# Bhasha-Open/Akshar

Hardware: AMD Instinct MI355X
Metric: MB of raw UTF-8 tokenized/sec @1 GPU (+ tokens/s); bit-exact vs CPU ref (higher is better)
Workload: dtype u8

## Files before the change

akshar_amd/csrc/ak_tile.h:

```cpp
#pragma once
#include <stddef.h>

#include "ak_dev.h"
#include "ak_ptc.h"
#include "ak_rows.h"
#include "ak_wave.h"

namespace ak {

#ifndef AK_T_BCAP
#define AK_T_BCAP 768
#endif
constexpr int T_BCAP = AK_T_BCAP;
constexpr int T_MAXR = 16;
#ifndef AK_TILE_UNIT
#define AK_TILE_UNIT 64
#endif
#ifndef AK_KNOCKOUT
#define AK_KNOCKOUT 0
#endif
#ifndef AK_TILE_WIDE
#define AK_TILE_WIDE 29
#endif
constexpr int TW_D1 = 1, TW_N = 4, TW_F = 8, TW_NS = 16;
// ... 388 lines not shown
    const bool dcand = ok && !(h & H_STABLE) && nfc_d_cand(h, hprev);
    uint32_t first = 0u;
    bool cand2 = false;
    if (lcand) {
        const uint32_t pi = hot_index(ppcp);
        const uint32_t pph = H[pi < HOT_N ? pi : 0u];
        cand2 = pi < HOT_N && (pph >> H_CCC_SHIFT) == 0u && !(pph & H_EXP);
        first = ppcp;
    } else if (dcand) {
        const uint2 pr = prop_global(pcp);
        cand2 = ((pr.y >> 16) & 7u) == 2u;
        first = cand2 ? AK_UT_DECOMP[pr.y >> 19] : 0u;
    }
    lok = cand2 && compose_pair<NF_UCD>(first, cp) == 0u;
    if ((lane == 0 && carry_cmp) || (lane == 1 && (carry_cmp & 2u))) lok = false;
#if AK_D2_SWAP
    const uint32_t hpp = w_prev(hprev, H_ROWSTART);
    const uint32_t hnx = w_next(h, H_ROWSTART);
    const bool ncmp = w_next((uint32_t)cmp, 1u) != 0u;
    const bool pok = w_prev((uint32_t)ok, 0u) != 0u;
    const uint32_t cm = h >> H_CCC_SHIFT, cpv = hprev >> H_CCC_SHIFT;
    const uint32_t cnx = (hnx & (H_STABLE | H_EXP)) ? 0u : (hnx >> H_CCC_SHIFT);
    bool scand = ok && pok && !cmp && !pfb && !lok && lane >= 1 && lane <= 62 && !(h & (H_STABLE | H_DECOMP)) &&
                 hprev != H_ROWSTART && !(hprev & (H_STABLE | H_DECOMP)) && cm != 0u && cm < cpv &&
                 (hpp == H_ROWSTART || (hpp >> H_CCC_SHIFT) == 0u) && (cnx == 0u || cnx >= cpv) && !ncmp &&
                 !(lane == 1 && (carry_cmp & 2u));
    if (w_ballot(scand && (h & H_SECOND))) {
        if (scand && (h & H_SECOND) && compose_pair<NF_UCD>(ppcp, cp) != 0u) scand = false;
    }
    const uint32_t mvn = w_next(mv), mvp = w_prev(mv, 0u);
    const bool sfirst = w_next((uint32_t)scand) != 0u;
    if (scand) {
        mv = mvp;
        lok = true;
    }
    if (sfirst) mv = mvn;
#endif
    const uint32_t cnext = w_next(cmp ? (cmv | 0x10000u) : 0u);
    if (cmp) mv = 0u;
    if (cnext) mv = cnext & 0xFFFFu;
    if (cmp && lane == 0) M.v[vpos - 1] = (uint16_t)cmv;
    const uint32_t cmp_hi = (uint32_t)(w_ballot(cmp) >> 62);
    return D2Exact{hp, hprev, mv, cmp_hi, pfb, lok};
}

template <int BCAP, class Mem, bool NFCD = false, int WIDE = 0>
__device__ __forceinline__ TileRows tile_front(const RowArgs &a, uint64_t r0, uint64_t rend, const uint32_t *H, Mem &M,
                                               bool raw = false) {
    const bool RAW = NFCD && raw;
    const int lane = w_lane();
    const int nr0 = (int)(rend - r0);
    const uint64_t myoff = lane <= nr0 ? a.offs[r0 + lane] : 0ull;
    const uint64_t S0 = w_bcast(myoff, 0);
    const bool fits = lane >= 1 && lane <= nr0 && (myoff - S0) <= (uint64_t)BCAP;
    const int k = w_popc(w_ballot(fits));
    const int nr = k ? k : 1;
    const uint64_t S1 = w_bcast(myoff, k);
    const uint64_t a0 = S0 & ~15ull;
    {
        const uint64_t nblk = (S1 - a0 + 15) / 16;
        const uint4 *src = (const uint4 *)(a.in) + a0 / 16;
        uint4 *dst = (uint4 *)M.bytes;
        for (uint64_t b = (uint64_t)lane; b < nblk; b += 64) dst[b] = src[b];
    }
    const uint64_t nextoff = w_shfl(myoff, lane + 1);
    if (lane < nr) {
        M.fb[lane] = lane >= k ? 1 : 0;
        M.rowend[lane] = (uint16_t)(nextoff - a0);
    }
    w_sync();

    if (AK_KNOCKOUT == 8) return TileRows{k, nr, S0, a0, 0u};
    uint16_t *P = M.w;
    uint32_t np = 0;
    bool swept = false;
    if constexpr ((WIDE & TW_D1) != 0) {
        static_assert(BCAP + 16 + 128 <= 32 * 32 && sizeof(M.v) >= 32 * 4, "the row-start bitmap: 32 dwords of V");
        const int s = lane < k ? (int)(myoff - a0) : 0;
        const uint32_t fbyte = M.bytes[s];
        swept = k > 0 && !w_ballot(lane < k && (nextoff == myoff || (fbyte & 0xC0u) == 0x80u));
        if (swept) {
            uint32_t *BM = (uint32_t *)M.v;
            if (lane < 32) BM[lane] = 0u;
            w_sync();
            if (lane < k) w_lds_or32(&BM[s >> 5], 1u << (s & 31));
            w_sync();
            const int s0 = (int)(S0 - a0), end = (int)(S1 - a0);
            const uint16_t *B2 = (const uint16_t *)M.bytes;
            uint16_t *dummy = M.w + (sizeof(M.w) / 2 - 64) + lane;
            for (int base = s0 & ~1; base < end; base += 128) {
                const int p0 = base + 2 * lane;
                const int pc = p0 < (end & ~1) ? p0 : (end & ~1);
                const uint32_t bb = B2[pc >> 1];
                const uint32_t mk = (BM[p0 >> 5] >> (p0 & 31)) & 3u;
                const bool l0 = p0 >= s0 && p0 < end && (bb & 0xC0u) != 0x80u;
                const bool l1 = p0 + 1 < end && (bb & 0xC000u) != 0x8000u;
                const uint32_t m0 = mk & 1u, m1 = mk >> 1;
                const uint32_t n0 = (uint32_t)l0 + m0;
                uint32_t tot;
                const uint32_t at = np + w_exscan(n0 + (uint32_t)l1 + m1, &tot);
                *(m0 ? &P[at] : dummy) = 0x8000u;
                *(l0 ? &P[at + m0] : dummy) = (uint16_t)p0;
                *(m1 ? &P[at + n0] : dummy) = 0x8000u;
                *(l1 ? &P[at + n0 + m1] : dummy) = (uint16_t)(p0 + 1);
                np += tot;
            }
        }
    }
    for (int i = 0; i < (swept ? 0 : k); ++i) {
        const int s = (int)(w_bcast(myoff, i) - a0), e = (int)(w_bcast(myoff, i + 1) - a0);
        if (lane == 0) P[np] = 0x8000u;
        ++np;
        bool bad_row = false;
        for (int base = s; base < e; base += 64) {
            const int p = base + lane;
            const bool in = p < e;
            const uint32_t b = in ? M.bytes[p] : 0u;
            const bool lead = in && (b & 0xC0u) != 0x80u;
            if (w_ballot(in && !lead && p == s)) { bad_row = true; break; }
            const uint64_t LM = w_ballot(lead);
            if (lead) P[np + w_rank(LM)] = (uint16_t)p;
            np += (uint32_t)w_popc(LM);
        }
        if (bad_row && lane == 0) M.fb[i] = 1;
    }
    w_sync();

    if (AK_KNOCKOUT == 9) return TileRows{k, nr, S0, a0, 0u};
    static_assert(sizeof(M.w) / 2 - 64 >= (size_t)(BCAP + T_MAXR + 1), "D2 dummy slots overlap P");
    uint16_t *dummy = M.w + (sizeof(M.w) / 2 - 64) + lane;
    uint32_t vpos = 0;
    {
        uint32_t carry_h = H_ROWSTART, rows = 0;
        uint32_t carry_cmp = 0;
        const uint32_t plast = np ? np - 1 : 0;
        const uint32_t hn_deva = H[0x093Cu - 0x900u + HOT_LO], hn_beng = H[0x09BCu - 0x900u + HOT_LO];
        for (uint32_t c0 = 0; c0 < np; c0 += 64) {
            const uint32_t c = c0 + lane;
            const bool in = c < np;
            const uint32_t ent0 = P[in ? c : plast];
            const uint32_t nent0 = P[c + 1 < np ? c + 1 : plast];
            const uint32_t ent = in ? ent0 : 0x8000u;
            const bool mark = in && (ent & 0x8000u);
            const uint64_t RMK = w_ballot(mark);
            const int row = (int)(rows + w_rank_incl(RMK)) - 1;
            const bool chr = in && !mark;
            const int pos = (int)(ent & 0x7FFFu);
            const int rend = (int)M.rowend[row > 0 ? row : 0];
            const uint32_t cp = decode_word(lds_word(M.bytes, pos), pos, rend);
            const uint32_t nent = c + 1 < np ? nent0 : 0x8000u;
            const int nxt = (nent & 0x8000u) ? rend : (int)nent;
#if AK_D2_BITWISE
            const bool bad = chr & ((cp == 0xFFFFFFFFu) | (pos + utf8_len(cp) != nxt) | (RAW & (cp >= V_SPECIAL)));
#else
            const bool bad = chr && (cp == 0xFFFFFFFFu || pos + utf8_len(cp) != nxt || (RAW && cp >= V_SPECIAL));
#endif
            const uint32_t ci = cp < HOT_LO ? cp : (cp - 0x900u < 0x100u ? cp - 0x900u + HOT_LO : 0u);
            uint32_t hw = H[ci];
#if AK_D2_BITWISE
            const bool cold = chr & !bad & (ci == 0u) & (cp != 0u);
#else
            const bool cold = chr && !bad && ci == 0u && cp != 0u;
#endif
            if (w_ballot(cold)) {
                if (cold) hw = hot_word(cp);
            }
            const uint32_t h = chr ? (bad ? 0u : hw) : H_ROWSTART;
            const bool xp = !RAW && chr && (h & H_EXP);
            uint32_t hp = xp ? ((h & 0xFFFFu) < 0x0980u ? hn_deva : hn_beng) : h;
            uint32_t hprev = w_prev(hp, carry_h);
            uint32_t mv = RAW ? (chr && !bad ? cp : 0u) : (chr ? (h & 0xFFFFu) : 0u);
#if AK_D2_BITWISE
            const bool ok = chr & !bad & !xp;
            const bool t0 = !NFCD && (ok & ((h & H_STABLE) == 0u) & nfc_trig_bf<false>(h, hprev));
            const bool pc = !NFCD && (ok & (hprev != H_ROWSTART) & ((h & H_SECOND) != 0u) & ((hprev & H_FIRST) != 0u));
#else
            const bool ok = chr && !bad && !xp;
            const bool t0 = !NFCD && ok && !(h & H_STABLE) && nfc_trig<false>(h, hprev);
            const bool pc = !NFCD && ok && nfc_pair_cand(h, hprev);
#endif
            uint32_t cmp_hi = 0;
            if (w_ballot(bad || t0 || pc)) {
                bool pfb = false, lok = false;
                if (AK_KNOCKOUT != 15 && !NFCD) {
                    const D2Exact r = d2_exact(M, P, H, c0, rows, vpos, carry_h, carry_cmp, h, cp, ok, chr, hp, hprev, mv);
                    hp = r.hp;
                    hprev = r.hprev;
                    mv = r.mv;
                    pfb = r.pfb;
                    lok = r.lok;
                    cmp_hi = r.cmp_hi;
                }
                const bool trig = bad || pfb || (!NFCD && ok && !(h & H_STABLE) && !lok && nfc_trig<false>(h, hprev));
                if (trig) M.fb[row] = 1;
            }
            const bool two = mark && row > 0;
            const uint32_t cnt = mark ? (two ? 2u : 1u) : (mv ? (xp ? 2u : 1u) : 0u);
            uint32_t tot;
            const uint32_t ex = w_exscan(cnt, &tot);
            uint16_t *d0 = cnt ? &M.v[vpos + ex] : dummy;
            uint16_t *d1 = (two || xp) ? &M.v[vpos + ex + 1] : dummy;
            *d0 = mark ? (two ? V_E : V_B) : (uint16_t)mv;
            *d1 = two ? V_B : (uint16_t)nukta_of(mv);
            vpos += tot;
            rows += (uint32_t)w_popc(RMK);
            carry_h = w_bcast(hp, 63);
            carry_cmp = cmp_hi;
        }
        if (k > 0) {
            if (lane == 0) M.v[vpos] = V_E;
            ++vpos;
        }
    }
    w_sync();
    return TileRows{k, nr, S0, a0, vpos};
}

__device__ __forceinline__ uint4 load_x4(const uint4 *p) {
#ifdef AK_HOST_EMU
    return *p;
#else
    typedef unsigned int u32x4 __attribute__((ext_vector_type(4)));
    const u32x4 v = *(const u32x4 *)p;
    return make_uint4(v.x, v.y, v.z, v.w);
#endif
}
__device__ __forceinline__ uint32_t ptc_probe(const BpeDev &m, bool cand, uint32_t n, const uint32_t q[7]) {
    const uint4 *tab = (const uint4 *)m.ptc;
    const uint32_t h = akp::ptc_hash(n, q[0], q[1], q[2], q[3], q[4], q[5], q[6]);
    const uint32_t s1 = akp::ptc_slot1(h, m.ptc_mask), s2 = akp::ptc_slot2(h, m.ptc_mask);
    const uint4 a = load_x4(tab + 2 * s1);
    bool m1 = cand & (((a.x >> 16) & 15u) == n) & (a.y == q[0]) & (a.z == q[1]) & (a.w == q[2]);
    if (w_ballot(m1 && n > 6)) {
        const uint4 b = load_x4(tab + 2 * s1 + 1);
        m1 = m1 & ((n <= 6) | ((b.x == q[3]) & (b.y == q[4]) & (b.z == q[5]) & (b.w == q[6])));
    }
    uint32_t res = m1 ? (a.x & 0xFFFFu) : 0xFFFFFFFFu;
    const bool try2 = cand & !m1 & ((a.x & akp::PTC_FLAG) != 0u);
    if (w_ballot(try2)) {
        const uint4 c = load_x4(tab + 2 * s2);
        bool m2 = try2 & (((c.x >> 16) & 15u) == n) & (c.y == q[0]) & (c.z == q[1]) & (c.w == q[2]);
        if (w_ballot(m2 && n > 6)) {
            const uint4 d = load_x4(tab + 2 * s2 + 1);
            m2 = m2 & ((n <= 6) | ((d.x == q[3]) & (d.y == q[4]) & (d.z == q[5]) & (d.w == q[6])));
        }
        res = m2 ? (c.x & 0xFFFFu) : res;
    }
    return res;
}


#ifndef AK_POOL_NCLASS
#define AK_POOL_NCLASS 1
#endif
constexpr int POOL_NCLASS = AK_POOL_NCLASS;
constexpr uint32_t POOL_RING = 320;
constexpr uint32_t POOL_CAP = POOL_NCLASS * POOL_RING;
#ifndef AK_POOL_INLINE
#define AK_POOL_INLINE 0
#endif
constexpr uint32_t POOL_U4 = POOL_CAP * (AK_POOL_INLINE ? 3u : 1u);
constexpr uint32_t STAGE_DEAD = 0xFFFFFFFFu;
static_assert(POOL_NCLASS == 1 || POOL_NCLASS == 4 || POOL_NCLASS == 8, "pool classes");
__device__ __forceinline__ uint32_t pool_class(uint32_t n) {
    if (POOL_NCLASS == 1) return 0u;
    if (POOL_NCLASS == 4) return n <= 3u ? 0u : n <= 5u ? 1u : n <= 8u ? 2u : 3u;
    return n <= 7u ? n - 2u : (n <= 9u ? 6u : 7u);
}

__device__ __forceinline__ uint4 load_l2(const uint4 *p) {
#ifdef AK_HOST_EMU
    return *p;
#else
    typedef unsigned int u32x4 __attribute__((ext_vector_type(4)));
    const u32x4 v = __builtin_nontemporal_load((const u32x4 *)p);
    return make_uint4(v.x, v.y, v.z, v.w);
#endif
}
__device__ __forceinline__ uint32_t load_l2(const uint32_t *p) {
#ifdef AK_HOST_EMU
    return *p;
#else
    return __builtin_nontemporal_load(p);
#endif
}

__device__ __forceinline__ void merge_rounds(const BpeDev &m, uint16_t *sym, uint16_t *rk16, uint32_t &alive,
                                             PassClock &pc) {
    for (;;) {
        if (AK_KNOCKOUT == 2) break;
        uint32_t e[WREG / 2];
        {
            const uint4 *r4 = (const uint4 *)rk16;
            const uint4 x0 = r4[0], x1 = r4[1];
            e[0] = x0.x; e[1] = x0.y; e[2] = x0.z; e[3] = x0.w; e[4] = x1.x; e[5] = x1.y; e[6] = x1.z; e[7] = x1.w;
        }
        const uint32_t m01 = pk_min_u16(e[0], e[1]), m23 = pk_min_u16(e[2], e[3]);
        const uint32_t m45 = pk_min_u16(e[4], e[5]), m67 = pk_min_u16(e[6], e[7]);
        const uint32_t mv = pk_min_u16(pk_min_u16(m01, m23), pk_min_u16(m45, m67));
        const uint32_t minv = (mv & 0xFFFFu) < (mv >> 16) ? (mv & 0xFFFFu) : (mv >> 16);
        const bool mg = minv != 0xFFFFu;
        if (!w_ballot(mg)) break;
        if (pc.on) {
            pc.count(TC_BROUNDS, 1);
            pc.count(TC_BLANES, w_ballot(mg));
        }
        if (mg) {
            const uint32_t mm = minv * 0x10001u;
            uint32_t one = 0x00010001u;
#ifndef AK_HOST_EMU
            asm volatile("" : "+v"(one));
#endif
            uint32_t kk[WREG / 2];
#pragma unroll
            for (int k = 0; k < WREG / 2; ++k)
                kk[k] = pk_mad_u16(pk_min_u16(e[k] ^ mm, one), 0x00100010u, (uint32_t)(2 * k) | ((uint32_t)(2 * k + 1) << 16));
            const uint32_t k01 = pk_min_u16(kk[0], kk[1]), k23 = pk_min_u16(kk[2], kk[3]);
            const uint32_t k45 = pk_min_u16(kk[4], kk[5]), k67 = pk_min_u16(kk[6], kk[7]);
            const uint32_t kmin = pk_min_u16(pk_min_u16(k01, k23), pk_min_u16(k45, k67));
            const int bi = (int)(((kmin & 0xFFFFu) < (kmin >> 16) ? kmin : (kmin >> 16)) & 15u);
            const uint32_t after = alive >> (bi + 1);
            const int jn = bi + 1 + __builtin_ctz(after);
            const uint32_t below = alive & ((1u << bi) - 1u);
            const int pl = below ? 31 - __builtin_clz(below) : -1;
            const uint32_t aj = jn + 1 < 32 ? alive >> (jn + 1) : 0u;
            const int q = aj ? jn + 1 + __builtin_ctz(aj) : -1;
            const uint32_t left = pl >= 0 ? sym[pl] : 0u;
            const uint32_t right = q >= 0 ? sym[q] : 0u;
            sym[bi] = (uint16_t)minv;
            alive &= ~(1u << jn);
            const uint32_t L = pl >= 0 ? merge_lookup_c(m, left, minv) & 0xFFFFu : 0xFFFFu;
            const uint32_t R = q >= 0 ? merge_lookup_c(m, minv, right) & 0xFFFFu : 0xFFFFu;
            if (pl >= 0) rk16[pl] = (uint16_t)L;
            rk16[bi] = (uint16_t)R;
            rk16[jn] = 0xFFFFu;
        }
    }
}

#ifndef AK_POOL_RB
#define AK_POOL_RB 1
#endif
#ifndef AK_POOL_WB
#define AK_POOL_WB 1
#endif
__device__ __forceinline__ void pool_flush(const TileArgs &ta, TileWaveMem &M, uint4 *pool, uint32_t c, uint32_t cnt,
                                           PassClock &pc) {
    static_assert(offsetof(TileWaveMem, bytes) == 0 && offsetof(TileWaveMem, w) + sizeof(TileWaveMem::w) >= 2 * 64 * 2 * WREG,
                  "rank rows + symbol rows fit the tile buffers");
    const BpeDev &m = ta.ra.bpe;
    const int lane = w_lane();
    const bool act = (uint32_t)lane < cnt;
    uint16_t *rk16 = (uint16_t *)((uint8_t *)&M + lane * (2 * WREG));
    uint16_t *sym = (uint16_t *)((uint8_t *)&M + 64 * 2 * WREG + lane * (2 * WREG));
#ifndef AK_HOST_EMU
    asm volatile("s_waitcnt vmcnt(0)" ::: "memory");
#endif
    uint4 *ring = pool + c * POOL_RING;
    const uint32_t head = w_bcast(M.phead[c], 0);
    const uint4 e = load_l2(ring + (head + (uint32_t)lane) % POOL_RING);
    const uint64_t dst = act ? (uint64_t)e.x | ((uint64_t)(e.y & 0xFFFFu) << 32) : 0ull;
    const int n = act ? (int)(e.y >> 16) : 0;
    const uint32_t row = e.z;
    uint32_t *sp = (uint32_t *)ta.ra.out + dst;
    uint32_t p[WREG / 2];
#if AK_POOL_INLINE
    {
        const uint4 *sy = pool + POOL_CAP + 2 * (c * POOL_RING + (head + (uint32_t)lane) % POOL_RING);
        const uint4 a = load_l2(sy), b = load_l2(sy + 1);
        p[0] = a.x; p[1] = a.y; p[2] = a.z; p[3] = a.w; p[4] = b.x; p[5] = b.y; p[6] = b.z; p[7] = b.w;
#pragma unroll
        for (int k = 0; k < WREG / 2; ++k) {
            const int i = 2 * k;
            p[k] = (i < n ? (p[k] & 0xFFFFu) : 0xFFFFu) | (i + 1 < n ? (p[k] & 0xFFFF0000u) : 0xFFFF0000u);
        }
    }
#else
    {
        const uint4 *s4 = (const uint4 *)sp;
#pragma unroll
        for (int k = 0; k < WREG / 4; ++k) {
            const uint4 v = (!AK_POOL_RB || k == 0 || w_ballot(4 * k < n)) ? load_l2(s4 + k) : make_uint4(0u, 0u, 0u, 0u);
            const uint32_t x[4] = {v.x, v.y, v.z, v.w};
#pragma unroll
            for (int h = 0; h < 2; ++h) {
                const int i = 4 * k + 2 * h;
                p[2 * k + h] = (i < n ? x[2 * h] : 0xFFFFu) | ((i + 1 < n ? x[2 * h + 1] : 0xFFFFu) << 16);
            }
        }
    }
#endif
    uint32_t d[WREG / 2];
#pragma unroll
    for (int k = 0; k < WREG / 2; ++k) {
        const int i = 2 * k;
        const uint32_t a0 = p[k] & 0xFFFFu, a1 = p[k] >> 16, a2 = k + 1 < WREG / 2 ? p[k + 1] & 0xFFFFu : 0xFFFFu;
        uint32_t l0 = 0xFFFFu, l1 = 0xFFFFu;
        if (AK_KNOCKOUT == 18 || i == 0 || w_ballot(i + 1 < n)) l0 = merge_lookup_c(m, a0, a1);
        if (i + 2 < WREG && (AK_KNOCKOUT == 18 || w_ballot(i + 2 < n))) l1 = merge_lookup_c(m, a1, a2);
        const uint32_t lo = i + 1 < n ? l0 & 0xFFFFu : 0xFFFFu;
        const uint32_t hi = (i + 2 < WREG && i + 2 < n) ? l1 & 0xFFFFu : 0xFFFFu;
        d[k] = lo | (hi << 16);
    }
    {
        uint4 *r4 = (uint4 *)rk16;
        r4[0] = make_uint4(d[0], d[1], d[2], d[3]);
        r4[1] = make_uint4(d[4], d[5], d[6], d[7]);
        uint4 *s4 = (uint4 *)sym;
        s4[0] = make_uint4(p[0], p[1], p[2], p[3]);
        s4[1] = make_uint4(p[4], p[5], p[6], p[7]);
    }
    if (pc.on) pc.count(TC_BBATCH, 1);
    uint32_t alive = act ? (1u << n) - 1u : 0u;
    merge_rounds(m, sym, rk16, alive, pc);
    {
        const uint4 *s4 = (const uint4 *)sym;
#pragma unroll
        for (int k = 0; k < WREG / 4; ++k) {
            const uint4 pr = s4[k / 2];
            const uint32_t w0 = (k & 1) ? pr.z : pr.x, w1 = (k & 1) ? pr.w : pr.y;
            uint32_t o[4];
#pragma unroll
            for (int t = 0; t < 4; ++t) {
                const int i = 4 * k + t;
                const uint32_t v = ((t < 2 ? w0 : w1) >> (16 * (t & 1))) & 0xFFFFu;
                o[t] = (alive >> i) & 1u ? v : STAGE_DEAD;
            }
#if AK_POOL_WB
            const int rem = n - 4 * k;
            if (rem >= 4) {
                ((uint4 *)sp)[k] = make_uint4(o[0], o[1], o[2], o[3]);
            } else if (rem == 3) {
#ifdef AK_HOST_EMU
                sp[4 * k] = o[0]; sp[4 * k + 1] = o[1]; sp[4 * k + 2] = o[2];
#else
                typedef unsigned int u32x3 __attribute__((ext_vector_type(3)));
                u32x3 v3;
                v3.x = o[0]; v3.y = o[1]; v3.z = o[2];
                *(u32x3 *)(sp + 4 * k) = v3;
#endif
            } else if (rem == 2) {
                *(uint2 *)(sp + 4 * k) = make_uint2(o[0], o[1]);
            } else if (rem == 1) {
                sp[4 * k] = o[0];
            }
#else
            if (4 * k + 3 < n) {
                ((uint4 *)sp)[k] = make_uint4(o[0], o[1], o[2], o[3]);
            } else {
#pragma unroll
                for (int t = 0; t < 3; ++t)
                    if (4 * k + t < n) sp[4 * k + t] = o[t];
            }
#endif
        }
    }
    const uint32_t dead = (uint32_t)n - (uint32_t)__builtin_popcount(alive);
    if (act && dead) atomicSub(ta.counts + row, dead);
    w_sync();
    if (lane == 0) {
        M.phead[c] = (head + cnt) % POOL_RING;
        M.pcnt[c] -= cnt;
    }
    w_sync();
}

__device__ __forceinline__ void unit_copy_live(const uint32_t *__restrict__ stage, uint64_t half, uint64_t base, uint64_t len,
                                               uint32_t *__restrict__ out, uint64_t cap, uint64_t d0, int lane) {
    constexpr int B = 4;
    uint64_t d = d0;
    for (uint64_t k0 = 0; k0 < len; k0 += 64 * B) {
        uint32_t v[B];
#pragma unroll
        for (int q = 0; q < B; ++q) {
            const uint64_t k = k0 + (uint64_t)(q * 64 + lane);
            v[q] = k < len && base + k < half ? stage[base + k] : STAGE_DEAD;
        }
#pragma unroll
        for (int q = 0; q < B; ++q) {
            const bool keep = v[q] != STAGE_DEAD;
            const uint64_t KM = w_ballot(keep);
            const uint64_t at = d + w_rank(KM);
            if (keep && at < cap) out[at] = v[q];
            d += (uint64_t)w_popc(KM);
        }
    }
}

__device__ __forceinline__ void pool_drain(const TileArgs &ta, TileWaveMem &M, uint4 *pool, uint32_t minc, PassClock &pc) {
#pragma unroll 1
    for (uint32_t c = 0; c < (uint32_t)POOL_NCLASS; ++c) {
        for (;;) {
            const uint32_t k = w_bcast(M.pcnt[c], 0);
            if (k < minc || k == 0) break;
            pool_flush(ta, M, pool, c, k < 64u ? k : 64u, pc);
        }
    }
}

template <int FLAGS, bool NFCD = false, int WIDE = 0>
__device__ __forceinline__ int bpe_tile(const TileArgs &ta, uint64_t r0, uint64_t rend, const uint32_t *H, const uint16_t *sfast,
                        TileWaveMem &M, uint4 *pool, PassClock &pc, bool raw = false) {
    const bool RAW = NFCD && raw;
    static_assert(FLAGS == 3, "the tile path implements normalize_text with its defaults");
    const int lane = w_lane();
    const RowArgs &a = ta.ra;
    const BpeDev &m = a.bpe;
    pc.mark(TP_STAGE);
    const TileRows tr = tile_front<T_BCAP, TileWaveMem, NFCD, WIDE>(a, r0, rend, H, M, raw);
    const int nr = tr.nr;
    const uint32_t vlen = tr.vlen;
    if (AK_KNOCKOUT == 10) return nr;

    pc.mark(TP_D);
    uint32_t wlen = 0;
    uint32_t nw = 0;
    constexpr bool WNS = (WIDE & TW_NS) != 0, WN = (WIDE & TW_N) != 0 || WNS;
    static_assert(2 * (T_SCAP + 64) <= (int)sizeof(TileWaveMem::bytes), "the start list + pass N's dummy slots in the staged bytes");
    uint16_t *const slist = (uint16_t *)M.bytes;
    if constexpr (WN) {
        uint16_t *dummy = (uint16_t *)M.bytes + (WNS ? T_SCAP : 0) + lane;
        const uint32_t *V32 = (const uint32_t *)M.v;
        const uint32_t h_sp = H[0x20];
        uint32_t carry_h = H_ROWSTART, carry_word = 0, carry_kword = 0xFFFFFFFFu, carry_ks = 0, rs = 0;
        const uint32_t dlast = (vlen ? vlen - 1 : 0) >> 1;
        auto cls_of = [](uint32_t h) -> uint32_t { return h == H_ROWSTART ? (uint32_t)HF_S : ((h >> H_CLS_SHIFT) & 3u); };
        for (uint32_t base = 0; base < vlen; base += 128) {
            const uint32_t k0 = base + 2u * (uint32_t)lane;
            const uint32_t d = k0 >> 1;
            const uint32_t dc = d < dlast ? d : dlast;
            const uint32_t wp = V32[dc >= 1 ? dc - 1 : 0], wx = V32[dc], wn = V32[dc < dlast ? dc + 1 : dlast];
            const bool in0 = k0 < vlen, in1 = k0 + 1 < vlen;
            const bool hasp = in0 && k0 >= 2;
            const uint32_t x0 = in0 ? (wx & 0xFFFFu) : (uint32_t)V_DEAD, x1 = in1 ? (wx >> 16) : (uint32_t)V_DEAD;
            const uint32_t pa0 = hasp ? (wp >> 16) : (uint32_t)V_DEAD, pb0 = hasp ? (wp & 0xFFFFu) : (uint32_t)V_DEAD;
            const uint32_t nx1 = k0 + 2 < vlen ? (wn & 0xFFFFu) : (uint32_t)V_DEAD;
            const bool sp0 = x0 >= V_SPECIAL, sp1 = x1 >= V_SPECIAL;
            const bool drop0 = !RAW && in0 && !sp0 && x0 != (uint32_t)'\n' && x0 == pa0 && (pa0 == pb0 || x1 == x0);
            const bool drop1 = !RAW && in1 && !sp1 && x1 != (uint32_t)'\n' && x1 == x0 && (x0 == pa0 || nx1 == x1);
            const bool keep0 = in0 && !drop0, keep1 = in1 && !drop1;
            const uint32_t xi0 = x0 < HOT_LO ? x0 : (x0 - 0x900u < 0x100u ? x0 - 0x900u + HOT_LO : 0u);
            const uint32_t xi1 = x1 < HOT_LO ? x1 : (x1 - 0x900u < 0x100u ? x1 - 0x900u + HOT_LO : 0u);
            uint32_t h0 = H[xi0], h1 = H[xi1];
            const bool cold0 = !sp0 && xi0 == 0u && x0 != 0u, cold1 = !sp1 && xi1 == 0u && x1 != 0u;
            if (w_ballot(cold0 || cold1)) {
                if (cold0) h0 = hot_of(prop_global(x0));
                if (cold1) h1 = hot_of(prop_global(x1));
            }
            h0 = sp0 ? H_ROWSTART : h0;
            h1 = sp1 ? H_ROWSTART : h1;
            const bool hs0 = !sp0 && (h0 & H_HFSPACE), hs1 = !sp1 && (h1 & H_HFSPACE);
            const uint32_t c0 = hs0 ? 0x20u : x0, c1 = hs1 ? 0x20u : x1;
            h0 = hs0 ? h_sp : h0;
            h1 = hs1 ? h_sp : h1;
            const uint32_t cls0 = cls_of(h0), cls1 = cls_of(h1);
            const uint64_t lt = w_lanemask_lt();
            const uint64_t pk = w_ballot(keep0 || keep1) & lt;
            const uint32_t h_l = w_shfl(keep1 ? h1 : h0, pk ? msb64(pk) : 0);
            const uint32_t hprev0 = pk ? h_l : carry_h;
            const uint32_t hprev1 = keep0 ? h0 : hprev0;
            const bool hfc0 = keep0 && !sp0 && !(h0 & H_HFST), hfc1 = keep1 && !sp1 && !(h1 & H_HFST);
            const bool trig0 = hfc0 && nfc_trig<true>(h0, hprev0), trig1 = hfc1 && nfc_trig<true>(h1, hprev1);
            const bool hpc0 = hfc0 && nfc_pair_cand(h0, hprev0), hpc1 = hfc1 && nfc_pair_cand(h1, hprev1);
            const bool wc0 = keep0 && !sp0 && cls0 != (uint32_t)HF_S, wc1 = keep1 && !sp1 && cls1 != (uint32_t)HF_S;
            const uint32_t st0 = wc0 && cls0 != cls_of(hprev0), st1 = wc1 && cls1 != cls_of(hprev1);
            const uint32_t si0 = sfast_index(c0), si1 = sfast_index(c1);
            uint32_t id0 = sfast[si0 < SFAST_N ? si0 : 0u], id1 = sfast[si1 < SFAST_N ? si1 : 0u];
            const bool rare0 = wc0 && si0 >= SFAST_N, rare1 = wc1 && si1 >= SFAST_N;
            if (w_ballot(rare0 || rare1)) {
                if (rare0) id0 = single_id_of(m, sfast, a.single_fast, c0);
                if (rare1) id1 = single_id_of(m, sfast, a.single_fast, c1);
            }
            id0 = wc0 ? id0 : 0xFFFFu;
            id1 = wc1 ? id1 : 0xFFFFu;
            const bool kept0 = id0 != 0xFFFFu, kept1 = id1 != 0xFFFFu;
            const uint32_t out0 = kept0 || (keep0 && sp0), out1 = kept1 || (keep1 && sp1);
            const uint32_t rm0 = keep0 && (x0 == V_B || x0 == V_FB), rm1 = keep1 && (x1 == V_B || x1 == V_FB);
            uint32_t tot;
            const uint32_t ex = w_exscan((st0 + st1) | ((out0 + out1) << 8) | ((rm0 + rm1) << 16), &tot);
            if (!RAW && w_ballot(trig0 || hpc0 || trig1 || hpc1)) {
                const uint32_t rrow0 = rs + (ex >> 16) + rm0 - 1u, rrow1 = rrow0 + rm1;
                if (trig0 || (hpc0 && compose_pair<NF_HFK>(hprev0 & 0xFFFFu, c0))) M.fb[rrow0] |= 2;
                if (trig1 || (hpc1 && compose_pair<NF_HFK>(hprev1 & 0xFFFFu, c1))) M.fb[rrow1] |= 2;
            }
            const uint32_t word0 = carry_word + (ex & 0xFFu) + st0, word1 = word0 + st1;
            const uint64_t pk2 = w_ballot(kept0 || kept1) & lt;
            const int src2 = pk2 ? msb64(pk2) : 0;
            const uint32_t kw_l = w_shfl(kept1 ? word1 : word0, src2);
            const uint32_t kprev0 = pk2 ? kw_l : carry_kword;
            const uint32_t kprev1 = kept0 ? word0 : kprev0;
            const bool ks0 = kept0 && word0 != kprev0, ks1 = kept1 && word1 != kprev1;
            const uint32_t pos0 = wlen + ((ex >> 8) & 0xFFu), pos1 = pos0 + out0;
            *(out0 ? &M.w[pos0] : dummy) = sp0 ? (uint16_t)x0 : (uint16_t)(id0 | (ks0 ? WSTART : 0u));
            *(out1 ? &M.w[pos1] : dummy) = sp1 ? (uint16_t)x1 : (uint16_t)(id1 | (ks1 ? WSTART : 0u));
            if constexpr (WNS) {
                const uint32_t ks_l = w_shfl((uint32_t)(kept1 ? ks1 : ks0), src2);
                const uint32_t pks0 = pk2 ? ks_l : carry_ks;
                const uint32_t pks1 = kept0 ? (uint32_t)ks0 : pks0;
                const uint32_t m0 = kept0 && !ks0 && pks0, m1 = kept1 && !ks1 && pks1;
                uint32_t mtot;
                const uint32_t j0 = nw + w_exscan(m0 + m1, &mtot), j1 = j0 + m0;
                *(m0 && j0 < (uint32_t)T_SCAP ? &slist[j0] : dummy) = (uint16_t)(pos0 - 1u);
                *(m1 && j1 < (uint32_t)T_SCAP ? &slist[j1] : dummy) = (uint16_t)(pos1 - 1u);
                nw += mtot;
                carry_ks = w_bcast((kept0 || kept1) ? (uint32_t)(kept1 ? ks1 : ks0) : pks0, 63);
            }
            wlen += (tot >> 8) & 0xFFu;
            rs += tot >> 16;
            carry_word += tot & 0xFFu;
            carry_h = w_bcast((keep0 || keep1) ? (keep1 ? h1 : h0) : hprev0, 63);
            carry_kword = w_bcast((kept0 || kept1) ? (kept1 ? word1 : word0) : kprev0, 63);
        }
    }
    {
        uint16_t *dummy = (uint16_t *)M.bytes;
        const uint32_t h_sp = H[0x20];
        uint32_t carry_h = H_ROWSTART, carry_word = 0, carry_kword = 0xFFFFFFFFu, rs = 0;
        int carry_cls = HF_S;
        const uint32_t vlast = vlen ? vlen - 1 : 0;
        for (uint32_t base = 0; base < (WN ? 0u : vlen); base += 64) {
            const uint32_t kk = base + lane;
            const bool in = kk < vlen;
            const uint32_t kc = in ? kk : vlast;
            const uint16_t x0 = M.v[kc];
            const uint16_t pa0 = M.v[kc >= 1 ? kc - 1 : 0];
            const uint16_t pb0 = M.v[kc >= 2 ? kc - 2 : 0];
            const uint16_t nx0 = M.v[kc + 1 < vlen ? kc + 1 : kc];
            uint16_t x = in ? x0 : V_DEAD;
            const uint16_t pa = in && kk >= 1 ? pa0 : V_DEAD;
            const uint16_t pb = in && kk >= 2 ? pb0 : V_DEAD;
            const uint16_t nx = in && kk + 1 < vlen ? nx0 : V_DEAD;
            const bool special = x >= V_SPECIAL;
#if AK_D2_BITWISE
            const bool drop = !RAW & in & !special & (x != (uint16_t)'\n') & (x == pa) & ((pa == pb) | (nx == x));
            const bool keep = in & !drop;
#else
            const bool drop = !RAW && in && !special && x != (uint16_t)'\n' && x == pa && (pa == pb || nx == x);
            const bool keep = in && !drop;
#endif
            const uint32_t xi = x < HOT_LO ? x : ((uint32_t)x - 0x900u < 0x100u ? (uint32_t)x - 0x900u + HOT_LO : 0u);
            uint32_t h = H[xi];
            const bool cold = !special && xi == 0u && x != 0;
            if (w_ballot(cold)) {
                if (cold) h = hot_of(prop_global(x));
            }
            h = special ? H_ROWSTART : h;
            const bool hsp = !special && (h & H_HFSPACE);
            x = hsp ? (uint16_t)0x20 : x;
            h = hsp ? h_sp : h;
            const int cls = special ? HF_S : (int)((h >> H_CLS_SHIFT) & 3u);
            const uint64_t KM = w_ballot(keep);
            const uint64_t lt = w_lanemask_lt();
            const uint64_t pk = KM & lt;
            const int src = pk ? msb64(pk) : 0;
            const uint32_t h_l = w_shfl(h, src);
            const int cls_l = w_shfl(cls, src);
            const uint32_t hprev = pk ? h_l : carry_h;
            const int cprev = pk ? cls_l : carry_cls;
            const uint64_t RM = w_ballot(keep && (x == V_B || x == V_FB));
#if AK_D2_BITWISE
            const bool hfc = keep & !special & ((h & H_HFST) == 0u);
            const bool trig = hfc & nfc_trig_bf<true>(h, hprev);
            const bool hpc = hfc & (hprev != H_ROWSTART) & ((h & H_SECOND) != 0u) & ((hprev & H_FIRST) != 0u);
#else
            const bool hfc = keep && !special && !(h & H_HFST);
            const bool trig = hfc && nfc_trig<true>(h, hprev);
            const bool hpc = hfc && nfc_pair_cand(h, hprev);
#endif
            if (!RAW && w_ballot(trig || hpc)) {
                const uint32_t rrow = rs + w_rank_incl(RM) - 1;
                if (trig || (hpc && compose_pair<NF_HFK>(hprev & 0xFFFFu, x))) M.fb[rrow] |= 2;
            }
#if AK_D2_BITWISE
            const bool wordchar = keep & !special & (cls != HF_S);
#else
            const bool wordchar = keep && !special && cls != HF_S;
#endif
            const uint64_t SM = w_ballot(wordchar && cls != cprev);
            const uint32_t word = carry_word + w_rank_incl(SM);
            const uint32_t si = sfast_index(x);
            uint32_t id = sfast[si < SFAST_N ? si : 0u];
            const bool rare = wordchar && si >= SFAST_N;
            if (w_ballot(rare)) {
                if (rare) id = single_id_of(m, sfast, a.single_fast, x);
            }
            id = wordchar ? id : 0xFFFFu;
            const bool kept = id != 0xFFFFu;
            const uint64_t K2 = w_ballot(kept);
            const uint64_t pk2 = K2 & lt;
            const uint32_t kw_l = w_shfl(word, pk2 ? msb64(pk2) : 0);
            const uint32_t kprev = pk2 ? kw_l : carry_kword;
            const bool kstart = kept && word != kprev;
            const bool out = kept || (keep && special);
            const uint64_t OM = w_ballot(out);
            uint16_t *dst = out ? &M.w[wlen + w_rank(OM)] : &dummy[lane];
            *dst = special ? x : (uint16_t)(id | (kstart ? WSTART : 0u));
            wlen += (uint32_t)w_popc(OM);
            rs += (uint32_t)w_popc(RM);
            if (KM) {
                const int lk = msb64(KM);
                carry_h = w_bcast(h, lk);
                carry_cls = w_bcast(cls, lk);
            }
            carry_word = w_bcast(word, 63);
            if (K2) carry_kword = w_bcast(word, msb64(K2));
        }
    }
    w_sync();

    pc.mark(TP_E);
    if (AK_KNOCKOUT == 11) return nr;
    for (uint32_t base = 0; base < (WNS ? 0u : wlen); base += 64) {
        const uint32_t kk = base + lane;
        const bool multi = kk + 1 < wlen && (M.w[kk] & 0x8000u) && M.w[kk] < V_SPECIAL && !(M.w[kk + 1] & 0x8000u);
// ... 273 lines not shown
```

Before: 134,100.

## Flatten pool-flush pair lookups across the wave via prefix-sum and bitmap

```diff
diff --git a/akshar_amd/csrc/ak_tile.h b/akshar_amd/csrc/ak_tile.h
--- a/akshar_amd/csrc/ak_tile.h
+++ b/akshar_amd/csrc/ak_tile.h
@@ -714,8 +714,12 @@
         const bool mg = minv != 0xFFFFu;
         if (!w_ballot(mg)) break;
         if (pc.on) {
+#if AK_POOL_STAT
+            pc.count(TC_BLANES, w_popc(w_ballot(mg)) <= 32 ? 1 : 0);
+#else
             pc.count(TC_BROUNDS, 1);
             pc.count(TC_BLANES, w_ballot(mg));
+#endif
         }
         if (mg) {
             const uint32_t mm = minv * 0x10001u;
@@ -756,12 +760,26 @@
 #ifndef AK_POOL_WB
 #define AK_POOL_WB 1
 #endif
+#ifndef AK_POOL_FLAT
+#define AK_POOL_FLAT 1
+#endif
+#ifndef AK_POOL_LANE_OPAQUE
+#define AK_POOL_LANE_OPAQUE AK_POOL_FLAT
+#endif
+#ifndef AK_POOL_STAT
+#define AK_POOL_STAT 0
+#endif
+constexpr int POOL_MARKW = 64 * (WREG - 2) / 32;
 __device__ __forceinline__ void pool_flush(const TileArgs &ta, TileWaveMem &M, uint4 *pool, uint32_t c, uint32_t cnt,
                                            PassClock &pc) {
-    static_assert(offsetof(TileWaveMem, bytes) == 0 && offsetof(TileWaveMem, w) + sizeof(TileWaveMem::w) >= 2 * 64 * 2 * WREG,
-                  "rank rows + symbol rows fit the tile buffers");
+    static_assert(offsetof(TileWaveMem, bytes) == 0 &&
+                      offsetof(TileWaveMem, w) + sizeof(TileWaveMem::w) >= 2 * 64 * 2 * WREG + (AK_POOL_FLAT ? 4 * POOL_MARKW : 0),
+                  "rank rows + symbol rows (+ the flat set-up's bitmap) fit the tile buffers");
     const BpeDev &m = ta.ra.bpe;
-    const int lane = w_lane();
+    int lane = w_lane();
+#if AK_POOL_LANE_OPAQUE && !defined(AK_HOST_EMU)
+    asm volatile("" : "+v"(lane));
+#endif
     const bool act = (uint32_t)lane < cnt;
     uint16_t *rk16 = (uint16_t *)((uint8_t *)&M + lane * (2 * WREG));
     uint16_t *sym = (uint16_t *)((uint8_t *)&M + 64 * 2 * WREG + lane * (2 * WREG));
@@ -802,6 +820,45 @@
         }
     }
 #endif
+#if AK_POOL_STAT
+    if (pc.on) {
+        uint32_t tot;
+        (void)w_exscan(n > 1 ? (uint32_t)n - 1u : 0u, &tot);
+        if (lane == 0) pc.acc[T_NPASS + TC_BROUNDS] += tot;
+    }
+#endif
+#if AK_POOL_FLAT
+    {
+        uint32_t P;
+        const uint32_t off = w_exscan(act ? (n > 1 ? (uint32_t)n - 1u : 1u) : 0u, &P);
+        uint4 *s4 = (uint4 *)sym;
+        s4[0] = make_uint4(p[0], p[1], p[2], p[3]);
+        s4[1] = make_uint4(p[4], p[5], p[6], (p[7] & 0xFFFFu) | (off << 16));
+        uint4 *r4 = (uint4 *)rk16;
+        r4[0] = make_uint4(~0u, ~0u, ~0u, ~0u);
+        r4[1] = make_uint4(~0u, ~0u, ~0u, ~0u);
+        uint32_t *marks = (uint32_t *)((uint8_t *)&M + 2 * 64 * 2 * WREG);
+        if (lane < POOL_MARKW) marks[lane] = 0u;
+        w_sync();
+        if (act) w_lds_or32(marks + (off >> 5), 1u << (off & 31u));
+        w_sync();
+        const uint16_t *syms = (const uint16_t *)((const uint8_t *)&M + 64 * 2 * WREG);
+        uint16_t *rks = (uint16_t *)&M;
+        uint32_t before = 0;
+#pragma unroll 1
+        for (uint32_t f0 = 0; f0 < P; f0 += 64u) {
+            const uint64_t S = (uint64_t)w_bcast(marks[f0 >> 5], 0) | ((uint64_t)w_bcast(marks[(f0 >> 5) + 1u], 0) << 32);
+            const bool real = f0 + (uint32_t)lane < P;
+            const uint32_t own = real ? before + w_rank_incl(S) - 1u : (uint32_t)lane;
+            const uint32_t pos = real ? f0 + (uint32_t)lane - syms[own * WREG + (WREG - 1)] : 0u;
+            const uint32_t a0 = syms[own * WREG + pos], a1 = syms[own * WREG + pos + 1u];
+            const uint32_t v = merge_lookup_c(m, a0, a1);
+            if (real && a1 != 0xFFFFu) rks[own * WREG + pos] = (uint16_t)v;
+            before += (uint32_t)w_popc(S);
+        }
+        w_sync();
+    }
+#else
     uint32_t d[WREG / 2];
 #pragma unroll
     for (int k = 0; k < WREG / 2; ++k) {
@@ -822,6 +879,7 @@
         s4[0] = make_uint4(p[0], p[1], p[2], p[3]);
         s4[1] = make_uint4(p[4], p[5], p[6], p[7]);
     }
+#endif
     if (pc.on) pc.count(TC_BBATCH, 1);
     uint32_t alive = act ? (1u << n) - 1u : 0u;
     merge_rounds(m, sym, rk16, alive, pc);
```

Measured after the change: 135,400 (median of 4 runs). No clear change (+1.0%).
